# EugenHotaj/zig_gpt2

Measured on AMD Instinct MI355X. Metric: tokens/sec GPT-2-124M greedy 1024-ctx, higher is better.
Workload: dtype bf16 weights, f32 activations/accumulate; 1 GPU; GPT-2 124M greedy decode, 1 prompt(s)/GPU x 1 GPU(s), 1-token prompts, 1024 decode steps per prompt (reference generate loop, src/main.zig:322-342); vocab=50257, context=1024, n_layer=12, n_heads=12, n_embed=768, prompts_per_gpu=1, global_prompts=1, kv_cache=f32, hip_graph=True, l2_prefetcher=on, parallelism=replicated weights, prompts sharded x1, RCCL broadcast at start-up only

## Files before the change

include/zgpt2.h:

```cpp
#ifndef ZGPT2_H
#define ZGPT2_H

#include <stddef.h>
#include <stdint.h>

#ifdef __cplusplus
extern "C" {
#endif

typedef enum {
    ZG_OK = 0,
    ZG_ERR_NOT_INITIALIZED = -1,
    ZG_ERR_SHAPE = -2,
    ZG_ERR_HIP = -3,
    ZG_ERR_STAGING = -4,
    ZG_ERR_UNSUPPORTED = -5,
    ZG_ERR_ARG = -6
} zg_status;


int zg_init(int device);
int zg_init_ex(int device, size_t staging_bytes);
int zg_shutdown(void);
const char* zg_last_error(void);
// ... 36 lines not shown

int zg_gelu(float* inputs, size_t inputs_len);

int zg_softmax(float* inputs, size_t inputs_len);

int zg_gemm_bf16_nt(const uint16_t* A, const uint16_t* B, const float* bias_or_null, void* C, size_t M,
                    size_t N, size_t K, int gelu, int out_bf16);
unsigned long long zg_debug_gemm_launches(void);
int zg_debug_gemm_stamps(unsigned long long* out, size_t n_words);
int zg_debug_prefill_linear(const uint16_t* A_planes, const uint16_t* W, const float* bias_or_null, void* C, size_t M, size_t N,
                            size_t K, int epilogue, int force_kernel, int slices, float* ws, size_t ws_floats);
int zg_debug_attn_prefill(const float* qkv, uint16_t* out, size_t batch, size_t n_tokens, size_t n_embed, size_t n_heads,
                          const float* k_cache, const float* v_cache, size_t ctx, float* ws, size_t ws_floats, int key_tiles);
int zg_debug_prefill_route(int force_kernel, int slices);
int zg_debug_last_kernel(char* out, size_t n);
int zg_f32_to_bf16(const float* src, uint16_t* dst_device, size_t len);


typedef struct {
    size_t vocab_size;
    size_t context_size;
    size_t n_layer;
    size_t n_heads;
    size_t n_embed;
} zg_gpt_config;

typedef struct zg_gpt zg_gpt;

enum {
    ZG_GPT_WEIGHTS_BF16 = 0,
// ... 87 lines not shown
```

zig_gpt2_amd/_lib.py:

```python
import ctypes as C
import os
import subprocess

_HERE = os.path.dirname(os.path.abspath(__file__))
CSRC = os.path.join(_HERE, "csrc")
SO_PATH = os.environ.get("ZGPT2_LIB") or os.path.join(_HERE, "lib", "libzgpt2_hip.so")
HEADER = os.path.join(os.path.dirname(_HERE), "include", "zgpt2.h")

_lib = None

f32p = C.POINTER(C.c_float)
szp = C.POINTER(C.c_size_t)
vp = C.c_void_p
sz = C.c_size_t


class ZgError(RuntimeError):
    def __init__(self, code, msg):
        super().__init__(f"libzgpt2_hip error {code}: {msg}")
        self.code = code


class GptConfig(C.Structure):

# ... 6 lines not shown


SIGNATURES = {
    "zg_init": (C.c_int, [C.c_int]),
    "zg_init_ex": (C.c_int, [C.c_int, sz]),
    "zg_shutdown": (C.c_int, []),
    "zg_last_error": (C.c_char_p, []),
    "zg_set_stream": (C.c_int, [vp]),
    "zg_synchronize": (C.c_int, []),
    "zg_register_tensor": (C.c_int, [vp, sz]),
    "zg_unregister_tensor": (C.c_int, [vp]),
    "zg_unregister_all": (C.c_int, []),
    "zg_debug_gemm_launches": (C.c_ulonglong, []),
    "zg_debug_gemm_stamps": (C.c_int, [vp, sz]),
    "zg_debug_last_kernel": (C.c_int, [C.c_char_p, sz]),
    "zg_debug_attn_prefill": (C.c_int, [vp, vp, sz, sz, sz, sz, vp, vp, sz, vp, sz, C.c_int]),
    "zg_debug_prefill_route": (C.c_int, [C.c_int, C.c_int]),
    "zg_debug_prefill_linear": (C.c_int, [vp, vp, vp, vp, sz, sz, sz, C.c_int, C.c_int, C.c_int, vp, sz]),
    "zg_linear_forward": (C.c_int, [sz, sz, vp, vp, vp, sz, vp, sz]),
    "zg_embedding_forward": (C.c_int, [sz, vp, sz, vp, sz, vp, sz]),
    "zg_layernorm_forward": (C.c_int, [sz, vp, vp, C.c_float, vp, sz]),
    "zg_attn_forward": (C.c_int, [sz, sz, vp, vp, vp, vp, sz, vp, sz] + [vp, sz] * 8),
    "zg_split_qkv": (C.c_int, [sz, sz, vp, sz, sz, vp, sz]),
    "zg_transpose": (C.c_int, [sz, sz, sz, vp, sz, vp, sz]),
    "zg_scaled_dot_product_attention": (C.c_int, [vp, sz, vp, sz, vp, sz, sz, sz, sz, vp, sz, vp, sz]),
    "zg_gemm_bf16_nt": (C.c_int, [vp, vp, vp, vp, sz, sz, sz, C.c_int, C.c_int]),
    "zg_f32_to_bf16": (C.c_int, [vp, vp, sz]),
    "zg_gelu": (C.c_int, [vp, sz]),
    "zg_softmax": (C.c_int, [vp, sz]),
    "zg_gpt_create": (C.c_int, [C.POINTER(vp), C.POINTER(GptConfig), sz, C.c_uint]),
# ... 88 lines not shown
```

zig_gpt2_amd/csrc/api_gpt.hip:

```cpp
#include <stdio.h>
#include <stdlib.h>
#include <string.h>

#include <string>
#include <thread>
#include <vector>

#include "zg_runtime.h"

using namespace zg;

struct zg_layer {
    void *c_attn_w, *c_proj_w, *c_fc_w, *mlp_proj_w;
    bf16_t *c_attn_p, *c_proj_p, *c_fc_p, *mlp_proj_p;
    float *c_attn_c2, *c_attn_c3, *c_fc_c2, *c_fc_c3;
    float *ln_1_g, *ln_1_b, *c_attn_b, *c_proj_b, *ln_2_g, *ln_2_b, *c_fc_b, *mlp_proj_b;
    void *k_cache, *v_cache;
};

struct zg_gpt {
    zg_gpt_config cfg;
    size_t batch;
    unsigned flags;
    int wt;
// ... 18 lines not shown
    unsigned sk_epoch;
    bool sk_used;
    bf16_t *pf_a, *pf_h;
    bf16_t *xp, *hp, *ap;
    int* attn_cnt;
    unsigned* epoch;
    unsigned spin_limit;
    unsigned* fault;
    unsigned long long *sk_tag, *part_tag;
    size_t sk_tag_bytes, part_tag_bytes;
    size_t epochs_since_clear;
    bool tags_on;
    unsigned long long* qkv_tag;
    size_t qkv_tag_bytes;
    bool fused_on;
    float* xst;
    bool st_on;
    bool pl_on;
    int max_splits, lm_grid;
    StepCtrl* h_ctrl;
    int* h_ints;
    std::vector<hipGraphExec_t> graphs;
    size_t n_buckets;
    int* sampled;
    float* samp_ws;
    SampleParams* samp;
    SampleParams* h_samp;
    bool gen_sampled;
    size_t graph_steps;
    hipStream_t graph_stream;
// ... 106 lines not shown
    g->out_tokens = (int*)P(B * C * 4);
    g->sampled = (int*)P(B * 4);
    g->samp = (SampleParams*)P(sizeof(SampleParams));
    g->samp_ws = (float*)P(sample_workspace_floats((int)B) * 4);
    g->xp = (bf16_t*)P(E * 48);
    g->hp = (bf16_t*)P(4 * E * 48);
    g->ap = (bf16_t*)P(E * 48);
    g->attn_cnt = (int*)P(8 * c.n_heads * 4);
    g->epoch = (unsigned*)P(256);
    g->xst = (float*)P(((E + 15) / 16) * 8 * 2 * 4);
    g->sk_tag_bytes = ((E + 15) / 16) * 4 * 128 * 8;
    g->part_tag_bytes = 8 * c.n_heads * g->max_splits * kPartStride * 8;
    g->sk_tag = (unsigned long long*)P(g->sk_tag_bytes);
    g->qkv_tag_bytes = 3 * E * 8;
    g->qkv_tag = (unsigned long long*)P(g->qkv_tag_bytes);
    g->part_tag = (unsigned long long*)P(g->part_tag_bytes);
    g->sk_tiles = (int)((E + 15) / 16);
    g->sk_ws = (float*)P((size_t)g->sk_tiles * 4 * 128 * 4);
    g->sk_cnt = (int*)P((size_t)g->sk_tiles * 4 * 4);
    g->pf_njobs = (int)(2 + 5 * L);
    g->pf_ctl = (PfCtl*)P(sizeof(PfCtl));
    g->pf_jobs = (PfJob*)P((size_t)g->pf_njobs * sizeof(PfJob));
    g->pf_x = g->pf_qkv = g->pf_ws = nullptr;
    g->sk_flags = nullptr;
    g->sk_epoch = 0;
    g->sk_used = false;
    g->pf_a = g->pf_h = nullptr;
    g->pf_ws_floats = 0;
    if (!(g->flags & ZG_GPT_NO_PREFILL)) {
        g->pf_x = (float*)P(B * C * E * 4);
// ... 48 lines not shown
    e.vocab = (int)g->cfg.vocab_size;
    e.prompt = g->prompt;
    e.prompt_stride = (int)g->cfg.context_size;
    e.prompt_len = g->prompt_len;
    e.forced = g->forced;
    e.cur_token = g->cur_token;
    e.out_tokens = g->out_tokens;
    e.out_stride = (int)g->cfg.context_size;
    e.part_val = g->part_val;
    e.part_idx = g->part_idx;
    e.part_stride = g->lm_grid;
    e.n_partials = g->lm_grid;
    e.x = g->x;
    e.pl_out = g->pl_on ? g->xp : nullptr;
    e.pl_g = g->layers[0].ln_1_g;
    e.epoch = (((g->pl_on && g->tags_on) || g->fused_on) && finish_only != 1 && finish_only != 2) ? g->epoch : nullptr;
    e.st_out = g->st_on ? g->xst : nullptr;
    e.finish_only = finish_only;
    e.progress = g->pf_on ? &g->pf_ctl->progress : nullptr;
    e.sampled = g->sampled;
    return e;
}

int emit_gemv(const zg_gpt* g, const GemvArgs& a, int grid, hipStream_t s, std::vector<PfJob>* rec, unsigned cls) {
    if (!rec) return launch_gemv(a, g->wt, grid, s);
    PfJob j{};
    j.cls = cls;
    const int rows = gemv_rows_per_wg(a, g->wt);
    if (rows > 0) {
        j.kind = PF_WEIGHTS;
        j.base = reinterpret_cast<const char*>(a.W);
// ... 243 lines not shown
            if (rec) {
                PfJob j{};
                j.kind = PF_KV;
                j.cls = 2;
                j.base = reinterpret_cast<const char*>(y.k_cache);
                j.base2 = reinterpret_cast<const char*>(y.v_cache);
                j.n_heads = (unsigned)g->cfg.n_heads;
                j.ctx = (unsigned)g->cfg.context_size;
                j.batch = (unsigned)g->batch;
                j.row_bytes = g->kv_mode ? 128u : 256u;
                rec->push_back(j);
            } else
                ZG_TRY(launch_attn_decode(a, s));
            ZG_TRY(prof_mark(prof, 2, s));
        }
        if (only < 0 || only == 3) ZG_TRY(gemv(c_proj_args(g, y, t_hi), 3));
        if (only < 0 || only == 4) ZG_TRY(gemv(c_fc_args(g, y, t_hi), 4));
        if (only < 0 || only == 5) {
            GemvArgs a = mlp_proj_args(g, l, t_hi);
            if (a.sk_tag) a.launch_id = launch_id(l, 1);
            ZG_TRY(gemv(a, 5));
        }
    }
    if (with_logits && (only < 0 || only == 6)) {
        ZG_TRY(enqueue_lm_head(g, s, rec));
        ZG_TRY(prof_mark(prof, 6, s));
    }
    if (o.with_sampler && with_logits && only < 0 && !rec)
        ZG_TRY(launch_sample_step(g->logits, (int)g->batch, (int)g->cfg.vocab_size, g->samp, g->ctrl, g->part_val, g->lm_grid, g->lm_grid, g->samp_ws,
                                  g->sampled, s));
    return ZG_OK;
}
// ... 28 lines not shown
                                   g->pf_ws_floats, nullptr, s, nullptr, np));
        const bool more = l + 1 < L;
        const PrefillLn ln1{more ? g->layers[l + 1].ln_1_g : nullptr, more ? g->layers[l + 1].ln_1_b : nullptr, 1e-5f, g->pf_a};
        ZG_TRY(launch_prefill_gemm(g->pf_h, f32w ? y.mlp_proj_p : (const bf16_t*)y.mlp_proj_w, y.mlp_proj_b, g->pf_x, M, iE, 4 * iE, iE, PF_RESID, g->pf_ws,
                                   g->pf_ws_floats, more ? &ln1 : nullptr, s, nullptr, np));
    }
    return ZG_OK;
}

int check_fault(zg_gpt* g) {
    unsigned sk = 0, tag = 0;
    if (g->sk_used) {
        g->sk_used = false;
        ZG_TRY(gemm_s4_fault(&sk));
    }
    if (g->tags_on || g->fused_on) {
        volatile unsigned* f = g->fault;
        tag = *f;
        if (tag) *f = 0;
    }
    if (sk) {
        set_error("a half-tile hand-over of the whole-prompt c_attn GEMM timed out%s: results discarded", tag ? " (and a tagged hand-over of the decode step)" : "");
        return ZG_ERR_HIP;
    }
    if (tag) {
        set_error("a tagged hand-over of the decode step timed out (a workgroup waited %u polls for its writers): results discarded", g->spin_limit);
        return ZG_ERR_HIP;
    }
    return ZG_OK;
}

int note_steps(zg_gpt* g, size_t n, hipStream_t s) {
    if (!g->tags_on && !g->fused_on) return ZG_OK;
    g->epochs_since_clear += n;
    if (g->epochs_since_clear < ((size_t)1 << 23)) return ZG_OK;
    g->epochs_since_clear = n;
    ZG_HIP(hipMemsetAsync(g->sk_tag, 0, g->sk_tag_bytes, s));
    ZG_HIP(hipMemsetAsync(g->part_tag, 0, g->part_tag_bytes, s));
    ZG_HIP(hipMemsetAsync(g->qkv_tag, 0, g->qkv_tag_bytes, s));
    return ZG_OK;
}

int setup_prefetcher(zg_gpt* g) {
    const bool small = g->stream == nullptr && g->batch == 1 && 4 * g->cfg.n_embed * g->cfg.n_embed * g->wbytes <= ((size_t)6 << 20);
    const int want = env_int("ZGPT2_PREFETCH", small ? 1 : 0);
    if ((g->flags & ZG_GPT_NO_PREFETCH) || !want || gs(g) == nullptr) return ZG_OK;
    if (g->pf_njobs > 255) return ZG_OK;
    std::vector<PfJob> jobs;
    StepOpts describe;
    describe.rec = &jobs;
    ZG_TRY(enqueue_step(g, true, (int)g->cfg.context_size, nullptr, describe));
    ZG_REQUIRE((int)jobs.size() == g->pf_njobs, ZG_ERR_ARG, "prefetcher: %zu launches per step", jobs.size());
    ZG_HIP(hipMemcpy(g->pf_jobs, jobs.data(), jobs.size() * sizeof(PfJob), hipMemcpyHostToDevice));
    int least = 0, greatest = 0;
// ... 246 lines not shown
    }
    ZG_REQUIRE(gemv_supported(mlp_proj_args(g, 0, 0), g->wt), ZG_ERR_UNSUPPORTED,
               "batch %zu with n_embed %zu: %zu input rows of 4*n_embed floats do not fit the LDS (use a smaller batch)", batch, c.n_embed, batch);
    auto every_linear = [&](bool (*ok)(const GemvArgs&, int)) {
        return ok(c_attn_args(g, y, 0), g->wt) && ok(c_proj_args(g, y, 0), g->wt) && ok(c_fc_args(g, y, 0), g->wt) &&
               ok(mlp_proj_args(g, 0, 0), g->wt);
    };
    if (g->wt == WT_BF16 && batch >= 2 && !(decode_paths_off() & 1)) {
        g->pl_on = true;
        g->pl_on = c.n_embed % 32 == 0 && every_linear(gemv_planes_ok);
    }
    g->tags_on = g->pl_on && !(decode_paths_off() & 4);
    g->spin_limit = (unsigned)env_int("ZGPT2_TAG_SPIN_LIMIT", 1 << 20);
    g->fused_on = batch == 1 && !(decode_paths_off() & 64) && c.n_layer <= 127 &&
                  attn_qkv_ok(c_attn_args(g, y, 0), attn_args(g, y, (int)c.context_size));
    if (g->pl_on && !(decode_paths_off() & 8) && c.n_embed % 16 == 0 && c.n_embed / 16 <= 128) {
        g->st_on = true;
        g->st_on = every_linear(gemv_pl4_ok);
    }
    ZG_REQUIRE(g->lm_grid <= 4096, ZG_ERR_UNSUPPORTED, "lm_head grid %d exceeds the argmax partial buffer", g->lm_grid);
    e = hipHostMalloc(reinterpret_cast<void**>(&g->h_ctrl), sizeof(StepCtrl) + 512, hipHostMallocDefault);
    if (e == hipSuccess) e = hipHostMalloc(reinterpret_cast<void**>(&g->h_ints), (batch * c.context_size + batch) * sizeof(int), hipHostMallocDefault);
    if (e != hipSuccess) return hip_fail(e, "hipHostMalloc(control mirrors)", __FILE__, __LINE__);
    static_assert(sizeof(StepCtrl) + sizeof(SampleParams) <= 256, "the fault word sits 256 bytes behind the control mirror");
    g->h_samp = reinterpret_cast<SampleParams*>(reinterpret_cast<char*>(g->h_ctrl) + 128);
    g->fault = reinterpret_cast<unsigned*>(reinterpret_cast<char*>(g->h_ctrl) + 256);
    *g->fault = 0;
    {
        const int k = env_int("ZGPT2_GRAPH_STEPS", 8);
        g->graph_steps = (k == 2 || k == 4 || k == 8 || k == 16 || k == 32 || k == 64) ? (size_t)k : 1;
// ... 654 lines not shown
```

zig_gpt2_amd/csrc/api_ops.hip:

```cpp
#include <stdarg.h>
#include <stdio.h>
#include <stdlib.h>
#include <string.h>

#include <algorithm>

#include "zg_runtime.h"

namespace zg {

static thread_local char g_err[512] = "";

int decode_paths_off() {
    const char* e = getenv("ZGPT2_DECODE_PATHS_OFF");
    return e ? atoi(e) : 0;
}

void set_error(const char* fmt, ...) {
    va_list ap;
    va_start(ap, fmt);
    vsnprintf(g_err, sizeof(g_err), fmt, ap);
    va_end(ap);
}

static thread_local char g_kernel[160] = "";
void note_kernel(const char* fmt, ...) {
    va_list ap;
    va_start(ap, fmt);
    vsnprintf(g_kernel, sizeof(g_kernel), fmt, ap);
    va_end(ap);
}

int hip_fail(hipError_t e, const char* what, const char* file, int line) {
    set_error("HIP error %d (%s) at %s:%d: %s", (int)e, hipGetErrorString(e), file, line, what);
    (void)hipGetLastError();
    return ZG_ERR_HIP;
}

Ctx& ctx() {
    static Ctx c;
    return c;
}

int require_init() {
    ZG_REQUIRE(ctx().inited, ZG_ERR_NOT_INITIALIZED, "zg_init has not been called");
// ... 533 lines not shown

int zg_debug_prefill_route(int force_kernel, int slices) {
    ZG_REQUIRE(force_kernel >= 0 && (force_kernel <= 2 || force_kernel >= 16) && slices >= 0, ZG_ERR_ARG, "debug_prefill_route: arguments");
    prefill_force_route(force_kernel, slices);
    return ZG_OK;
}

unsigned long long zg_debug_gemm_launches(void) { return gemm_mfma_launch_count(); }
int zg_debug_gemm_stamps(unsigned long long* out, size_t n_words) { return gemm_debug_stamps(out, n_words); }
int zg_debug_last_kernel(char* out, size_t n) {
    if (!out || n == 0) return ZG_ERR_ARG;
    snprintf(out, n, "%s", zg::g_kernel);
    return ZG_OK;
}

int zg_f32_to_bf16(const float* src, uint16_t* dst_device, size_t len) {
    ZG_TRY(require_init());
    ZG_REQUIRE(src && dst_device && is_device_ptr(dst_device), ZG_ERR_ARG, "f32_to_bf16: bad argument");
    Call call;
    CallGuard guard(call);
    const float* s;
    ZG_TRY(call.in(src, len, &s));
    ZG_TRY(launch_f32_to_bf16(s, dst_device, len, call.stream()));
    ZG_TRY(call.finish());
    guard.done = true;
    return ZG_OK;
}

int zg_embedding_forward(size_t emb_dim, const float* weight, size_t weight_len, const size_t* idxs,
                         size_t idxs_len, float* embeddings, size_t embeddings_len) {
// ... 281 lines not shown
```

zig_gpt2_amd/csrc/gemv_internal.h:

```cpp
#pragma once
#include <stdlib.h>

#include "zg_kernels.h"

#ifdef ZG_STAMPS
#define ZG_STAMP_DECL() unsigned long long zg_ts[8] = {0, 0, 0, 0, 0, 0, 0, 0}
#define ZG_STAMP(i) zg_ts[i] = __builtin_amdgcn_s_memtime()
#define ZG_STAMP_FLUSH()                                                                              \
    if (a.dbg && threadIdx.x == 0 && (blockIdx.x == 0 || blockIdx.x == gridDim.x - 1)) {             \
        const unsigned long long slot = atomicAdd(a.dbg, 1ull);                                       \
        unsigned long long* d = a.dbg + 16 + slot * 10;                                               \
        for (int i = 0; i < 8; ++i) d[i] = zg_ts[i];                                                  \
        d[8] = blockIdx.x;                                                                            \
        d[9] = __builtin_amdgcn_s_memtime();                                                          \
    }
#else
#define ZG_STAMP_DECL()
#define ZG_STAMP(i)
#define ZG_STAMP_FLUSH()
#endif

namespace zg {

namespace {
// ... 358 lines not shown
    return a.kslices <= 1 && a.epilogue != EPI_ARGMAX && a.rows_per_wave == 1 && gemv_mfma_lds(a.K, 16) > 160 * 1024;
}

inline int pl4_pairs(const GemvArgs& a) {
    const int off = decode_paths_off() & 2;
    if (off || a.pl_in == nullptr || a.epilogue == EPI_ARGMAX || a.rows_per_wave != 1) return 0;
    if (a.N > 0xffff || (a.prologue == PRO_LAYERNORM && a.x_stride != a.K) || (a.epilogue == EPI_RESIDUAL && a.resid_stride != a.N)) return 0;
    if (a.st_in != nullptr && a.K / 16 > 128) return 0;
    const int ksl = a.kslices > 1 ? a.kslices : 1;
    if (a.K % (64 * ksl) != 0) return 0;
    const int kp = (a.K / ksl / 64 + 3) / 4;
    return kp <= 5 ? kp : 0;
}

template <typename WT, int LPR, int CPL, int NP, bool TAGGED>
__device__ __forceinline__ void gemv_lnk_body(int blk, const void* __restrict__ Wv, const float* __restrict__ xin, unsigned ne, int K,
                                              const float* __restrict__ ln_g, const float* __restrict__ c2, const float* __restrict__ c3,
                                              const int* __restrict__ cw, const GemvArgs& a, unsigned pf_inc,
                                              unsigned long long* __restrict__ tagw, const unsigned* __restrict__ ew, unsigned launch_id) {
    const int N = (int)(ne & 0xffffffu), epilogue = (int)(ne >> 24);
    ZG_STAMP_DECL();
    ZG_STAMP(0);
    constexpr int RPP = 64 / LPR, ROWS = NP * RPP;
    __shared__ float part[4][ROWS];
    __shared__ float stat[4][2];
    const int tid = threadIdx.x, lane = tid & 63;
    const int wave = __builtin_amdgcn_readfirstlane(tid >> 6);
    const int lr = lane % LPR, rsub = lane / LPR;
    int kbeg, nchq;
    if (sizeof(WT) == 2 && (K & 63) == 0 && ((K >> 6) & 3) != 0 && (((K >> 6) >> 2) + 1) * 8 <= LPR * CPL) {
        const int lines = K >> 6, base = lines >> 2, rem = lines & 3;
        kbeg = (wave * base + min(wave, rem)) * 64;
        nchq = (base + (wave < rem ? 1 : 0)) * 8;
    } else {
// ... 1 lines not shown
        nchq = K >> 5;
    }
    const auto W = wmat<WT>(Wv, kbeg);
    const int row0 = blk * ROWS;
    Raw<WT> wq[NP][CPL];
#pragma unroll
    for (int p = 0; p < NP; ++p) {
        const auto pr = wrow(W, (size_t)min(row0 + p * RPP + rsub, N - 1), K);
#pragma unroll
        for (int i = 0; i < CPL; ++i) wq[p][i] = load_raw(pr, min(lr + LPR * i, nchq - 1));
    }
    W8 xr[CPL], gr[CPL];
#pragma unroll
    for (int i = 0; i < CPL; ++i) {
        const size_t off = (size_t)kbeg + (size_t)min(lr + LPR * i, nchq - 1) * 8;
        xr[i] = load_x8(xin + off);
        gr[i] = load_x8(ln_g + off);
    }
    float c2n = 0.0f, c3n = 0.0f;
    if (tid < ROWS) {
        const int n = min(row0 + tid, N - 1);
        c2n = c2[n];
        c3n = c3[n];
    }
    const int T = max(cw[1], 1);
    const unsigned epoch = TAGGED ? ew[0] : 0u;
    ZG_STAMP(1);
    {
        ZG_PIN(a.progress); ZG_PIN(a.y); ZG_PIN(a.y_stride); ZG_PIN(a.epilogue); ZG_PIN(__float_as_uint(a.eps));
        if (epilogue == EPI_QKV) {
            ZG_PIN(a.q); ZG_PIN(a.k_cache); ZG_PIN(a.v_cache); ZG_PIN(a.N); ZG_PIN(a.head_dim); ZG_PIN(a.n_heads); ZG_PIN(a.ctx); ZG_PIN(a.kv_mode); ZG_PIN(a.kv_lo);
        }
    }
    if (TAGGED) { ZG_PIN(tagw); ZG_PIN(launch_id); }
    pf_count(a.progress, pf_inc);
    ZG_STAMP(2);
    float sx = 0.0f, sxx = 0.0f;
#pragma unroll
    for (int i = 0; i < CPL; ++i) {
        if (lr + LPR * i >= nchq) xr[i] = zero_w8();
#pragma unroll
        for (int j = 0; j < 8; ++j) {
            sx += xr[i].v[j];
            sxx = fmaf(xr[i].v[j], xr[i].v[j], sxx);
            xr[i].v[j] *= gr[i].v[j];
        }
    }
    sx = group_allsum<LPR>(sx);
    sxx = group_allsum<LPR>(sxx);
    auto dot = [&](const Raw<WT>(&w)[CPL]) {
// ... 59 lines not shown
```

zig_gpt2_amd/csrc/gemv_ksplit.hip:

```cpp
#include "gemv_internal.h"

namespace zg {

namespace {

template <typename WT, int LPR, int CPL, int NP = 2>
__global__ __launch_bounds__(256) void gemv_ksplit_kernel(const void* __restrict__ Wv, const float* __restrict__ xin, int N,
                                                          int K, unsigned em, const float* __restrict__ part_in, int max_splits,
                                                          const float* __restrict__ bias, const float* __restrict__ resid,
                                                          const GemvArgs a) {
    const int epilogue = (int)(em & 0xffu), merge_splits = (int)((em >> 8) & 0xffu);
    const int has_bias = (int)((em >> 16) & 1u), has_resid = (int)((em >> 17) & 1u);
    ZG_STAMP_DECL();
    ZG_STAMP(0);
    constexpr int RPP = 64 / LPR, ROWS = NP * RPP;
    __shared__ float part[4][ROWS];
    const int tid = threadIdx.x, lane = tid & 63;
    const int wave = __builtin_amdgcn_readfirstlane(tid >> 6);
    const int lr = lane % LPR, rsub = lane / LPR;
    const int Kq = K >> 2, nchq = Kq >> 3;
    const auto W = wmat<WT>(Wv, (size_t)wave * Kq);
    const int row0 = blockIdx.x * ROWS;
    Raw<WT> wq[NP][CPL];
#pragma unroll
    for (int p = 0; p < NP; ++p) {
        const auto pr = wrow(W, (size_t)min(row0 + p * RPP + rsub, N - 1), K);
#pragma unroll
        for (int i = 0; i < CPL; ++i) wq[p][i] = load_raw(pr, min(lr + LPR * i, nchq - 1));
    }
    W8 xr[CPL];
    if (merge_splits > 0) {
        constexpr int MAXS = 4;
        const int nsplit = merge_splits;
#pragma unroll
        for (int i = 0; i < CPL; ++i) {
            const int e0 = wave * Kq + min(lr + LPR * i, nchq - 1) * 8;
            const int h = e0 >> 6, d0 = e0 & 63;
            const float* p = part_in + ((size_t)h * max_splits) * kPartStride;
            float ms[MAXS], ls[MAXS];
            W8 o[MAXS];
#pragma unroll
            for (int sp = 0; sp < MAXS; ++sp) {
                const float* ps = p + min(sp, nsplit - 1) * kPartStride;
                ms[sp] = ps[64];
                ls[sp] = ps[65];
                const float2 a0 = *reinterpret_cast<const float2*>(ps + d0), a1 = *reinterpret_cast<const float2*>(ps + d0 + 2);
                const float2 a2 = *reinterpret_cast<const float2*>(ps + d0 + 4), a3 = *reinterpret_cast<const float2*>(ps + d0 + 6);
                o[sp].v[0] = a0.x; o[sp].v[1] = a0.y; o[sp].v[2] = a1.x; o[sp].v[3] = a1.y;
                o[sp].v[4] = a2.x; o[sp].v[5] = a2.y; o[sp].v[6] = a3.x; o[sp].v[7] = a3.y;
            }
#pragma unroll
            for (int sp = 0; sp < MAXS; ++sp)
                if (sp >= nsplit) ms[sp] = -1e30f;
            const float mx = fmaxf(fmaxf(ms[0], ms[1]), fmaxf(ms[2], ms[3]));
            float l = 0.0f;
            W8 r = zero_w8();
#pragma unroll
            for (int sp = 0; sp < MAXS; ++sp) {
                const float w = __expf(ms[sp] - mx);
                l = fmaf(w, ls[sp], l);
#pragma unroll
                for (int j = 0; j < 8; ++j) r.v[j] = fmaf(w, o[sp].v[j], r.v[j]);
            }
            const float inv = 1.0f / l;
#pragma unroll
            for (int j = 0; j < 8; ++j) xr[i].v[j] = r.v[j] * inv;
        }
    } else {
#pragma unroll
        for (int i = 0; i < CPL; ++i) xr[i] = load_x8(xin + (size_t)wave * Kq + (size_t)min(lr + LPR * i, nchq - 1) * 8);
    }
    float bias_n = 0.0f, resid_n = 0.0f;
    if (tid < ROWS) {
        const int n = min(row0 + tid, N - 1);
        bias_n = bias[n * has_bias];
        resid_n = resid[n * has_resid];
    }
    ZG_STAMP(1);
    ZG_PIN(a.y);
    ZG_PIN(a.progress);
    pf_count(a.progress);
    ZG_STAMP(2);
#pragma unroll
    for (int i = 0; i < CPL; ++i)
        if (lr + LPR * i >= nchq) xr[i] = zero_w8();
    auto dot = [&](const Raw<WT>(&w)[CPL]) {
        float p0 = 0.0f, p1 = 0.0f, p2 = 0.0f, p3 = 0.0f;
#pragma unroll
        for (int i = 0; i < CPL; ++i) {
            const W8 u = unpack(w[i]);
            p0 = fmaf(u.v[0], xr[i].v[0], p0); p1 = fmaf(u.v[1], xr[i].v[1], p1);
            p2 = fmaf(u.v[2], xr[i].v[2], p2); p3 = fmaf(u.v[3], xr[i].v[3], p3);
            p0 = fmaf(u.v[4], xr[i].v[4], p0); p1 = fmaf(u.v[5], xr[i].v[5], p1);
            p2 = fmaf(u.v[6], xr[i].v[6], p2); p3 = fmaf(u.v[7], xr[i].v[7], p3);
        }
        return group_allsum<LPR>((p0 + p1) + (p2 + p3));
    };
    float sp[NP];
#pragma unroll
    for (int p = 0; p < NP; ++p) sp[p] = dot(wq[p]);
    ZG_STAMP(3);
    if (lr == 0) {
#pragma unroll
        for (int p = 0; p < NP; ++p) part[wave][p * RPP + rsub] = sp[p];
    }
    __syncthreads();
    ZG_STAMP(4);
    if (tid < ROWS && row0 + tid < N) {
        const int n = row0 + tid;
        const float v = ((part[0][tid] + part[1][tid]) + (part[2][tid] + part[3][tid])) + bias_n;
        a.y[n] = epilogue == EPI_RESIDUAL ? v + resid_n : (epilogue == EPI_GELU ? gelu_ref(v) : v);
    }
    ZG_STAMP(5);
    ZG_STAMP(6);
    ZG_STAMP(7);
    ZG_STAMP_FLUSH();
}

template <typename WT>
int launch_ksplit(const GemvArgs& a, hipStream_t s) {
    const int nchq = a.K / 32;
    const int merge_splits = a.prologue == PRO_ATTN_MERGE ? (a.t_hi + kAttnChunk - 1) / kAttnChunk : 0;
    const unsigned has_resid = a.epilogue == EPI_RESIDUAL ? 1u : 0u;
    const unsigned em = (unsigned)a.epilogue | ((unsigned)merge_splits << 8) | ((a.bias ? 1u : 0u) << 16) | (has_resid << 17);
#define ZG_KS(LPR_, CPL_)                                                                                                \
    {                                                                                                                    \
        constexpr int rows = 2 * (64 / LPR_);                                                                            \
        note_kernel("gemv_ksplit_kernel<%s, %d, %d, 2>", wt_name<WT>(), LPR_, CPL_);         \
        hipLaunchKernelGGL((gemv_ksplit_kernel<WT, LPR_, CPL_, 2>), dim3((a.N + rows - 1) / rows), dim3(256), 0, s, a.W,     \
                           a.x,                                                                                         \
                           a.N, a.K, em, a.part ? a.part : a.zero, a.max_splits, a.bias ? a.bias : a.zero,              \
// ... 111 lines not shown
```

zig_gpt2_amd/csrc/zg_kernels.h:

```cpp
#pragma once
#include "zg_common.h"

namespace zg {

struct StepCtrl {
    int step;
    int seq_len;
    int mode;
    int n_partials;
};

enum GemvPrologue { PRO_NONE = 0, PRO_LAYERNORM = 1, PRO_ATTN_MERGE = 2 };
enum GemvEpilogue { EPI_STORE = 0, EPI_RESIDUAL = 1, EPI_GELU = 2, EPI_QKV = 3, EPI_ARGMAX = 4 };
enum WeightType { WT_BF16 = 0, WT_F32 = 1, WT_B24 = 2  };

constexpr int kAttnChunk = 256;
constexpr int kPartStride = 64 + 2;

struct GemvArgs {
    const void* W;
    const float* bias;
    int N, K, M;
    int rows_per_wave;
    int waves_per_wg;
// ... 66 lines not shown
    int t_hi;
    int max_splits;
    float* part;
    unsigned* progress;
    bf16_t* pl_out;
    int* merge_cnt;
    const unsigned* epoch;
    unsigned launch_id;
    unsigned long long* part_tag;
    unsigned* fault;
    unsigned spin_limit;
};
int launch_attn_decode(const AttnArgs& a, hipStream_t s);
bool attn_qkv_ok(const GemvArgs& g, const AttnArgs& at);
int launch_attn_qkv(const GemvArgs& g, int weight_type, const AttnArgs& at, const unsigned* epoch, unsigned long long* qkv_tag, hipStream_t s);
int launch_attn_any_dim(const float* q, const float* k, const float* v, long stride_b, long stride_h, long stride_t, int batch, int n_heads,
                        int head_dim, int seq_len, float* out, hipStream_t s);
int launch_attn_merge(const float* part, int batch, int n_heads, int head_dim, int max_splits,
                      int seq_len, float* out, hipStream_t s);

int launch_epoch_bump(unsigned* epoch, hipStream_t s);
int launch_layernorm(float* x, int rows, int n, const float* g, const float* b, float eps, hipStream_t s, unsigned* done_flag = nullptr,
                     unsigned done_seq = 0, bool* announced = nullptr, float* shadow = nullptr);
int launch_gelu(float* x, size_t n, hipStream_t s, unsigned* done_flag = nullptr, unsigned done_seq = 0, bool* announced = nullptr, float* shadow = nullptr);
int launch_softmax(float* x, size_t n, hipStream_t s, unsigned* done_flag = nullptr, unsigned done_seq = 0, bool* announced = nullptr);
int launch_done_flag(unsigned* flag, unsigned seq, hipStream_t s);
struct CopySegs {
    const void* src[4];
    void* dst[4];
    unsigned bytes[4];
// ... 165 lines not shown
```

Before: 5021 tokens/s.

## Fuse attention c_proj and MLP c_fc gemvs into one tagged launch

Adds a combined kernel in which the first blocks compute the attention output projection with residual and publish each output element with an epoch/launch tag. The remaining blocks run the layernorm+c_fc+GELU gemv, preload their weights, then spin on the tags instead of waiting for a kernel boundary. This removes one launch and one inter-kernel gap per layer and lets c_fc weight loads overlap c_proj. In exchange it relies on both block groups being co-resident, with a spin limit and fault flag as the fallback. Also factors the ksplit gemv body into a shared device function and adds a per-name kernel launch counter for debugging.

New measurement: 5016 tokens/s. Within noise of the previous version (-0.1%).

```diff
diff --git a/include/zgpt2.h b/include/zgpt2.h
--- a/include/zgpt2.h
+++ b/include/zgpt2.h
@@ -74,6 +74,7 @@
                           const float* k_cache, const float* v_cache, size_t ctx, float* ws, size_t ws_floats, int key_tiles);
 int zg_debug_prefill_route(int force_kernel, int slices);
 int zg_debug_last_kernel(char* out, size_t n);
+unsigned long long zg_debug_kernel_launches(const char* prefix);
 int zg_f32_to_bf16(const float* src, uint16_t* dst_device, size_t len);
 
 
diff --git a/zig_gpt2_amd/_lib.py b/zig_gpt2_amd/_lib.py
--- a/zig_gpt2_amd/_lib.py
+++ b/zig_gpt2_amd/_lib.py
@@ -44,6 +44,7 @@
     "zg_debug_gemm_launches": (C.c_ulonglong, []),
     "zg_debug_gemm_stamps": (C.c_int, [vp, sz]),
     "zg_debug_last_kernel": (C.c_int, [C.c_char_p, sz]),
+    "zg_debug_kernel_launches": (C.c_ulonglong, [C.c_char_p]),
     "zg_debug_attn_prefill": (C.c_int, [vp, vp, sz, sz, sz, sz, vp, vp, sz, vp, sz, C.c_int]),
     "zg_debug_prefill_route": (C.c_int, [C.c_int, C.c_int]),
     "zg_debug_prefill_linear": (C.c_int, [vp, vp, vp, vp, sz, sz, sz, C.c_int, C.c_int, C.c_int, vp, sz]),
diff --git a/zig_gpt2_amd/csrc/api_gpt.hip b/zig_gpt2_amd/csrc/api_gpt.hip
--- a/zig_gpt2_amd/csrc/api_gpt.hip
+++ b/zig_gpt2_amd/csrc/api_gpt.hip
@@ -56,6 +56,9 @@
     unsigned long long* qkv_tag;
     size_t qkv_tag_bytes;
     bool fused_on;
+    unsigned long long* x_tag;
+    size_t x_tag_bytes;
+    bool projfc_on;
     float* xst;
     bool st_on;
     bool pl_on;
@@ -192,6 +195,8 @@
     g->sk_tag = (unsigned long long*)P(g->sk_tag_bytes);
     g->qkv_tag_bytes = 3 * E * 8;
     g->qkv_tag = (unsigned long long*)P(g->qkv_tag_bytes);
+    g->x_tag_bytes = E * 8;
+    g->x_tag = (unsigned long long*)P(g->x_tag_bytes);
     g->part_tag = (unsigned long long*)P(g->part_tag_bytes);
     g->sk_tiles = (int)((E + 15) / 16);
     g->sk_ws = (float*)P((size_t)g->sk_tiles * 4 * 128 * 4);
@@ -270,7 +275,7 @@
     e.x = g->x;
     e.pl_out = g->pl_on ? g->xp : nullptr;
     e.pl_g = g->layers[0].ln_1_g;
-    e.epoch = (((g->pl_on && g->tags_on) || g->fused_on) && finish_only != 1 && finish_only != 2) ? g->epoch : nullptr;
+    e.epoch = (((g->pl_on && g->tags_on) || g->fused_on || g->projfc_on) && finish_only != 1 && finish_only != 2) ? g->epoch : nullptr;
     e.st_out = g->st_on ? g->xst : nullptr;
     e.finish_only = finish_only;
     e.progress = g->pf_on ? &g->pf_ctl->progress : nullptr;
@@ -544,8 +549,18 @@
                 ZG_TRY(launch_attn_decode(a, s));
             ZG_TRY(prof_mark(prof, 2, s));
         }
-        if (only < 0 || only == 3) ZG_TRY(gemv(c_proj_args(g, y, t_hi), 3));
-        if (only < 0 || only == 4) ZG_TRY(gemv(c_fc_args(g, y, t_hi), 4));
+        bool pf = false;
+        if (g->projfc_on && !g->pf_on && only < 0 && !rec && 2 * l + 1 <= 255) {
+            const GemvArgs p = c_proj_args(g, y, t_hi), c = c_fc_args(g, y, t_hi);
+            if (proj_fc_ok(p, c)) {
+                pf = true;
+                ZG_TRY(launch_proj_fc(p, c, g->wt, g->epoch, g->x_tag, g->fault, g->spin_limit, launch_id(l, 0), s));
+                ZG_TRY(prof_mark(prof, 3, s));
+                ZG_TRY(prof_mark(prof, 4, s));
+            }
+        }
+        if (!pf && (only < 0 || only == 3)) ZG_TRY(gemv(c_proj_args(g, y, t_hi), 3));
+        if (!pf && (only < 0 || only == 4)) ZG_TRY(gemv(c_fc_args(g, y, t_hi), 4));
         if (only < 0 || only == 5) {
             GemvArgs a = mlp_proj_args(g, l, t_hi);
             if (a.sk_tag) a.launch_id = launch_id(l, 1);
@@ -604,7 +619,7 @@
         g->sk_used = false;
         ZG_TRY(gemm_s4_fault(&sk));
     }
-    if (g->tags_on || g->fused_on) {
+    if (g->tags_on || g->fused_on || g->projfc_on) {
         volatile unsigned* f = g->fault;
         tag = *f;
         if (tag) *f = 0;
@@ -621,13 +636,14 @@
 }
 
 int note_steps(zg_gpt* g, size_t n, hipStream_t s) {
-    if (!g->tags_on && !g->fused_on) return ZG_OK;
+    if (!g->tags_on && !g->fused_on && !g->projfc_on) return ZG_OK;
     g->epochs_since_clear += n;
     if (g->epochs_since_clear < ((size_t)1 << 23)) return ZG_OK;
     g->epochs_since_clear = n;
     ZG_HIP(hipMemsetAsync(g->sk_tag, 0, g->sk_tag_bytes, s));
     ZG_HIP(hipMemsetAsync(g->part_tag, 0, g->part_tag_bytes, s));
     ZG_HIP(hipMemsetAsync(g->qkv_tag, 0, g->qkv_tag_bytes, s));
+    ZG_HIP(hipMemsetAsync(g->x_tag, 0, g->x_tag_bytes, s));
     return ZG_OK;
 }
 
@@ -904,6 +920,7 @@
     g->spin_limit = (unsigned)env_int("ZGPT2_TAG_SPIN_LIMIT", 1 << 20);
     g->fused_on = batch == 1 && !(decode_paths_off() & 64) && c.n_layer <= 127 &&
                   attn_qkv_ok(c_attn_args(g, y, 0), attn_args(g, y, (int)c.context_size));
+    g->projfc_on = batch == 1 && !(decode_paths_off() & 128) && c.n_layer <= 127 && proj_fc_ok(c_proj_args(g, y, 64), c_fc_args(g, y, 64));
     if (g->pl_on && !(decode_paths_off() & 8) && c.n_embed % 16 == 0 && c.n_embed / 16 <= 128) {
         g->st_on = true;
         g->st_on = every_linear(gemv_pl4_ok);
diff --git a/zig_gpt2_amd/csrc/api_ops.hip b/zig_gpt2_amd/csrc/api_ops.hip
--- a/zig_gpt2_amd/csrc/api_ops.hip
+++ b/zig_gpt2_amd/csrc/api_ops.hip
@@ -24,11 +24,23 @@
 }
 
 static thread_local char g_kernel[160] = "";
+struct KernelCount {
+    char name[160];
+    unsigned long long n;
+};
+static thread_local KernelCount g_kernel_counts[64];
 void note_kernel(const char* fmt, ...) {
     va_list ap;
     va_start(ap, fmt);
     vsnprintf(g_kernel, sizeof(g_kernel), fmt, ap);
     va_end(ap);
+    for (KernelCount& k : g_kernel_counts) {
+        if (k.n == 0) memcpy(k.name, g_kernel, sizeof(k.name));
+        if (strcmp(k.name, g_kernel) == 0) {
+            ++k.n;
+            break;
+        }
+    }
 }
 
 int hip_fail(hipError_t e, const char* what, const char* file, int line) {
@@ -592,6 +604,14 @@
     return ZG_OK;
 }
 
+unsigned long long zg_debug_kernel_launches(const char* prefix) {
+    unsigned long long n = 0;
+    if (prefix)
+        for (const zg::KernelCount& k : zg::g_kernel_counts)
+            if (k.n && strncmp(k.name, prefix, strlen(prefix)) == 0) n += k.n;
+    return n;
+}
+
 int zg_f32_to_bf16(const float* src, uint16_t* dst_device, size_t len) {
     ZG_TRY(require_init());
     ZG_REQUIRE(src && dst_device && is_device_ptr(dst_device), ZG_ERR_ARG, "f32_to_bf16: bad argument");
diff --git a/zig_gpt2_amd/csrc/gemv_internal.h b/zig_gpt2_amd/csrc/gemv_internal.h
--- a/zig_gpt2_amd/csrc/gemv_internal.h
+++ b/zig_gpt2_amd/csrc/gemv_internal.h
@@ -396,10 +396,131 @@
 }
 
 template <typename WT, int LPR, int CPL, int NP, bool TAGGED>
+__device__ __forceinline__ void gemv_ksplit_body(int blk, const void* __restrict__ Wv, const float* __restrict__ xin, int N, int K, unsigned em,
+                                                 const float* __restrict__ part_in, int max_splits, const float* __restrict__ bias,
+                                                 const float* __restrict__ resid, const GemvArgs& a, unsigned pf_inc,
+                                                 unsigned long long* __restrict__ tagw, const unsigned* __restrict__ ew, unsigned launch_id) {
+    const int epilogue = (int)(em & 0xffu), merge_splits = (int)((em >> 8) & 0xffu);
+    const int has_bias = (int)((em >> 16) & 1u), has_resid = (int)((em >> 17) & 1u);
+    ZG_STAMP_DECL();
+    ZG_STAMP(0);
+    constexpr int RPP = 64 / LPR, ROWS = NP * RPP;
+    __shared__ float part[4][ROWS];
+    const int tid = threadIdx.x, lane = tid & 63;
+    const int wave = __builtin_amdgcn_readfirstlane(tid >> 6);
+    const int lr = lane % LPR, rsub = lane / LPR;
+    const int Kq = K >> 2, nchq = Kq >> 3;
+    const auto W = wmat<WT>(Wv, (size_t)wave * Kq);
+    const int row0 = (int)((unsigned)blk * (unsigned)ROWS);
+    Raw<WT> wq[NP][CPL];
+#pragma unroll
+    for (int p = 0; p < NP; ++p) {
+        const auto pr = wrow(W, (size_t)min(row0 + p * RPP + rsub, N - 1), K);
+#pragma unroll
+        for (int i = 0; i < CPL; ++i) wq[p][i] = load_raw(pr, min(lr + LPR * i, nchq - 1));
+    }
+    W8 xr[CPL];
+    if (merge_splits > 0) {
+        constexpr int MAXS = 4;
+        const int nsplit = merge_splits;
+#pragma unroll
+        for (int i = 0; i < CPL; ++i) {
+            const int e0 = wave * Kq + min(lr + LPR * i, nchq - 1) * 8;
+            const int h = e0 >> 6, d0 = e0 & 63;
+            const float* p = part_in + ((size_t)h * max_splits) * kPartStride;
+            float ms[MAXS], ls[MAXS];
+            W8 o[MAXS];
+#pragma unroll
+            for (int sp = 0; sp < MAXS; ++sp) {
+                const float* ps = p + min(sp, nsplit - 1) * kPartStride;
+                ms[sp] = ps[64];
+                ls[sp] = ps[65];
+                const float2 a0 = *reinterpret_cast<const float2*>(ps + d0), a1 = *reinterpret_cast<const float2*>(ps + d0 + 2);
+                const float2 a2 = *reinterpret_cast<const float2*>(ps + d0 + 4), a3 = *reinterpret_cast<const float2*>(ps + d0 + 6);
+                o[sp].v[0] = a0.x; o[sp].v[1] = a0.y; o[sp].v[2] = a1.x; o[sp].v[3] = a1.y;
+                o[sp].v[4] = a2.x; o[sp].v[5] = a2.y; o[sp].v[6] = a3.x; o[sp].v[7] = a3.y;
+            }
+#pragma unroll
+            for (int sp = 0; sp < MAXS; ++sp)
+                if (sp >= nsplit) ms[sp] = -1e30f;
+            const float mx = fmaxf(fmaxf(ms[0], ms[1]), fmaxf(ms[2], ms[3]));
+            float l = 0.0f;
+            W8 r = zero_w8();
+#pragma unroll
+            for (int sp = 0; sp < MAXS; ++sp) {
+                const float w = __expf(ms[sp] - mx);
+                l = fmaf(w, ls[sp], l);
+#pragma unroll
+                for (int j = 0; j < 8; ++j) r.v[j] = fmaf(w, o[sp].v[j], r.v[j]);
+            }
+            const float inv = 1.0f / l;
+#pragma unroll
+            for (int j = 0; j < 8; ++j) xr[i].v[j] = r.v[j] * inv;
+        }
+    } else {
+#pragma unroll
+        for (int i = 0; i < CPL; ++i) xr[i] = load_x8(xin + (size_t)wave * Kq + (size_t)min(lr + LPR * i, nchq - 1) * 8);
+    }
+    float bias_n = 0.0f, resid_n = 0.0f;
+    if (tid < ROWS) {
+        const int n = min(row0 + tid, N - 1);
+        bias_n = bias[n * has_bias];
+        resid_n = resid[n * has_resid];
+    }
+    const unsigned epoch = TAGGED ? ew[0] : 0u;
+    ZG_STAMP(1);
+    ZG_PIN(a.y);
+    ZG_PIN(a.progress);
+    if (TAGGED) { ZG_PIN(tagw); ZG_PIN(launch_id); }
+    pf_count(a.progress, pf_inc);
+    ZG_STAMP(2);
+#pragma unroll
+    for (int i = 0; i < CPL; ++i)
+        if (lr + LPR * i >= nchq) xr[i] = zero_w8();
+    auto dot = [&](const Raw<WT>(&w)[CPL]) {
+        float p0 = 0.0f, p1 = 0.0f, p2 = 0.0f, p3 = 0.0f;
+#pragma unroll
+        for (int i = 0; i < CPL; ++i) {
+            const W8 u = unpack(w[i]);
+            p0 = fmaf(u.v[0], xr[i].v[0], p0); p1 = fmaf(u.v[1], xr[i].v[1], p1);
+            p2 = fmaf(u.v[2], xr[i].v[2], p2); p3 = fmaf(u.v[3], xr[i].v[3], p3);
+            p0 = fmaf(u.v[4], xr[i].v[4], p0); p1 = fmaf(u.v[5], xr[i].v[5], p1);
+            p2 = fmaf(u.v[6], xr[i].v[6], p2); p3 = fmaf(u.v[7], xr[i].v[7], p3);
+        }
+        return group_allsum<LPR>((p0 + p1) + (p2 + p3));
+    };
+    float sp[NP];
+#pragma unroll
+    for (int p = 0; p < NP; ++p) sp[p] = dot(wq[p]);
+    ZG_STAMP(3);
+    if (lr == 0) {
+#pragma unroll
+        for (int p = 0; p < NP; ++p) part[wave][p * RPP + rsub] = sp[p];
+    }
+    __syncthreads();
+    ZG_STAMP(4);
+    if (tid < ROWS && row0 + tid < N) {
+        const int n = row0 + tid;
+        const float v = ((part[0][tid] + part[1][tid]) + (part[2][tid] + part[3][tid])) + bias_n;
+        const float out = epilogue == EPI_RESIDUAL ? v + resid_n : (epilogue == EPI_GELU ? gelu_ref(v) : v);
+        a.y[n] = out;
+        if (TAGGED)
+            __hip_atomic_store(tagw + n, ((unsigned long long)((epoch << 8) | launch_id) << 32) | __float_as_uint(out), __ATOMIC_RELAXED,
+                               __HIP_MEMORY_SCOPE_AGENT);
+    }
+    ZG_STAMP(5);
+    ZG_STAMP(6);
+    ZG_STAMP(7);
+    ZG_STAMP_FLUSH();
+}
+
+template <typename WT, int LPR, int CPL, int NP, bool TAGGED, bool XT = false>
 __device__ __forceinline__ void gemv_lnk_body(int blk, const void* __restrict__ Wv, const float* __restrict__ xin, unsigned ne, int K,
                                               const float* __restrict__ ln_g, const float* __restrict__ c2, const float* __restrict__ c3,
                                               const int* __restrict__ cw, const GemvArgs& a, unsigned pf_inc,
-                                              unsigned long long* __restrict__ tagw, const unsigned* __restrict__ ew, unsigned launch_id) {
+                                              unsigned long long* __restrict__ tagw, const unsigned* __restrict__ ew, unsigned launch_id,
+                                              const unsigned long long* __restrict__ xtag = nullptr, unsigned xid = 0u,
+                                              unsigned* __restrict__ fault = nullptr, unsigned spin_limit = 0u) {
     const int N = (int)(ne & 0xffffffu), epilogue = (int)(ne >> 24);
     ZG_STAMP_DECL();
     ZG_STAMP(0);
@@ -431,7 +552,7 @@
 #pragma unroll
     for (int i = 0; i < CPL; ++i) {
         const size_t off = (size_t)kbeg + (size_t)min(lr + LPR * i, nchq - 1) * 8;
-        xr[i] = load_x8(xin + off);
+        if (!XT) xr[i] = load_x8(xin + off);
         gr[i] = load_x8(ln_g + off);
     }
     float c2n = 0.0f, c3n = 0.0f;
@@ -441,7 +562,7 @@
         c3n = c3[n];
     }
     const int T = max(cw[1], 1);
-    const unsigned epoch = TAGGED ? ew[0] : 0u;
+    const unsigned epoch = (TAGGED || XT) ? ew[0] : 0u;
     ZG_STAMP(1);
     {
         ZG_PIN(a.progress); ZG_PIN(a.y); ZG_PIN(a.y_stride); ZG_PIN(a.epilogue); ZG_PIN(__float_as_uint(a.eps));
@@ -451,6 +572,39 @@
     }
     if (TAGGED) { ZG_PIN(tagw); ZG_PIN(launch_id); }
     pf_count(a.progress, pf_inc);
+    if constexpr (XT) {
+        constexpr int QW = LPR * CPL * 8, NX = QW / 64;
+        __shared__ __attribute__((aligned(16))) float xs[4][QW];
+        ZG_PIN(xtag); ZG_PIN(xid); ZG_PIN(fault); ZG_PIN(spin_limit);
+        const unsigned tag = (epoch << 8) | xid;
+        const int nw = nchq * 8;
+        const unsigned long long* src = xtag + kbeg;
+        unsigned long long wv[NX];
+#pragma unroll
+        for (int j = 0; j < NX; ++j) wv[j] = 0ull;
+        for (unsigned spins = 0;; ++spins) {
+            bool ok = true;
+#pragma unroll
+            for (int j = 0; j < NX; ++j) {
+                if (64 * j < nw) {
+                    wv[j] = __hip_atomic_load(src + min(lane + 64 * j, nw - 1), __ATOMIC_RELAXED, __HIP_MEMORY_SCOPE_AGENT);
+                    ok = ok && (unsigned)(wv[j] >> 32) == tag;
+                }
+            }
+            if (__builtin_amdgcn_ballot_w64(!ok) == 0) break;
+            if (spins >= spin_limit) {
+                if (lane == 0 && fault) __hip_atomic_store(fault, 1u, __ATOMIC_RELAXED, __HIP_MEMORY_SCOPE_AGENT);
+                break;
+            }
+            __builtin_amdgcn_s_sleep(1);
+        }
+#pragma unroll
+        for (int j = 0; j < NX; ++j)
+            if (lane + 64 * j < nw) xs[wave][lane + 64 * j] = __uint_as_float((unsigned)wv[j]);
+        __builtin_amdgcn_wave_barrier();
+#pragma unroll
+        for (int i = 0; i < CPL; ++i) xr[i] = load_x8(&xs[wave][min(lr + LPR * i, nchq - 1) * 8]);
+    }
     ZG_STAMP(2);
     float sx = 0.0f, sxx = 0.0f;
 #pragma unroll
diff --git a/zig_gpt2_amd/csrc/gemv_ksplit.hip b/zig_gpt2_amd/csrc/gemv_ksplit.hip
--- a/zig_gpt2_amd/csrc/gemv_ksplit.hip
+++ b/zig_gpt2_amd/csrc/gemv_ksplit.hip
@@ -9,112 +9,7 @@
                                                           int K, unsigned em, const float* __restrict__ part_in, int max_splits,
                                                           const float* __restrict__ bias, const float* __restrict__ resid,
                                                           const GemvArgs a) {
-    const int epilogue = (int)(em & 0xffu), merge_splits = (int)((em >> 8) & 0xffu);
-    const int has_bias = (int)((em >> 16) & 1u), has_resid = (int)((em >> 17) & 1u);
-    ZG_STAMP_DECL();
-    ZG_STAMP(0);
-    constexpr int RPP = 64 / LPR, ROWS = NP * RPP;
-    __shared__ float part[4][ROWS];
-    const int tid = threadIdx.x, lane = tid & 63;
-    const int wave = __builtin_amdgcn_readfirstlane(tid >> 6);
-    const int lr = lane % LPR, rsub = lane / LPR;
-    const int Kq = K >> 2, nchq = Kq >> 3;
-    const auto W = wmat<WT>(Wv, (size_t)wave * Kq);
-    const int row0 = blockIdx.x * ROWS;
-    Raw<WT> wq[NP][CPL];
-#pragma unroll
-    for (int p = 0; p < NP; ++p) {
-        const auto pr = wrow(W, (size_t)min(row0 + p * RPP + rsub, N - 1), K);
-#pragma unroll
-        for (int i = 0; i < CPL; ++i) wq[p][i] = load_raw(pr, min(lr + LPR * i, nchq - 1));
-    }
-    W8 xr[CPL];
-    if (merge_splits > 0) {
-        constexpr int MAXS = 4;
-        const int nsplit = merge_splits;
-#pragma unroll
-        for (int i = 0; i < CPL; ++i) {
-            const int e0 = wave * Kq + min(lr + LPR * i, nchq - 1) * 8;
-            const int h = e0 >> 6, d0 = e0 & 63;
-            const float* p = part_in + ((size_t)h * max_splits) * kPartStride;
-            float ms[MAXS], ls[MAXS];
-            W8 o[MAXS];
-#pragma unroll
-            for (int sp = 0; sp < MAXS; ++sp) {
-                const float* ps = p + min(sp, nsplit - 1) * kPartStride;
-                ms[sp] = ps[64];
-                ls[sp] = ps[65];
-                const float2 a0 = *reinterpret_cast<const float2*>(ps + d0), a1 = *reinterpret_cast<const float2*>(ps + d0 + 2);
-                const float2 a2 = *reinterpret_cast<const float2*>(ps + d0 + 4), a3 = *reinterpret_cast<const float2*>(ps + d0 + 6);
-                o[sp].v[0] = a0.x; o[sp].v[1] = a0.y; o[sp].v[2] = a1.x; o[sp].v[3] = a1.y;
-                o[sp].v[4] = a2.x; o[sp].v[5] = a2.y; o[sp].v[6] = a3.x; o[sp].v[7] = a3.y;
-            }
-#pragma unroll
-            for (int sp = 0; sp < MAXS; ++sp)
-                if (sp >= nsplit) ms[sp] = -1e30f;
-            const float mx = fmaxf(fmaxf(ms[0], ms[1]), fmaxf(ms[2], ms[3]));
-            float l = 0.0f;
-            W8 r = zero_w8();
-#pragma unroll
-            for (int sp = 0; sp < MAXS; ++sp) {
-                const float w = __expf(ms[sp] - mx);
-                l = fmaf(w, ls[sp], l);
-#pragma unroll
-                for (int j = 0; j < 8; ++j) r.v[j] = fmaf(w, o[sp].v[j], r.v[j]);
-            }
-            const float inv = 1.0f / l;
-#pragma unroll
-            for (int j = 0; j < 8; ++j) xr[i].v[j] = r.v[j] * inv;
-        }
-    } else {
-#pragma unroll
-        for (int i = 0; i < CPL; ++i) xr[i] = load_x8(xin + (size_t)wave * Kq + (size_t)min(lr + LPR * i, nchq - 1) * 8);
-    }
-    float bias_n = 0.0f, resid_n = 0.0f;
-    if (tid < ROWS) {
-        const int n = min(row0 + tid, N - 1);
-        bias_n = bias[n * has_bias];
-        resid_n = resid[n * has_resid];
-    }
-    ZG_STAMP(1);
-    ZG_PIN(a.y);
-    ZG_PIN(a.progress);
-    pf_count(a.progress);
-    ZG_STAMP(2);
-#pragma unroll
-    for (int i = 0; i < CPL; ++i)
-        if (lr + LPR * i >= nchq) xr[i] = zero_w8();
-    auto dot = [&](const Raw<WT>(&w)[CPL]) {
-        float p0 = 0.0f, p1 = 0.0f, p2 = 0.0f, p3 = 0.0f;
-#pragma unroll
-        for (int i = 0; i < CPL; ++i) {
-            const W8 u = unpack(w[i]);
-            p0 = fmaf(u.v[0], xr[i].v[0], p0); p1 = fmaf(u.v[1], xr[i].v[1], p1);
-            p2 = fmaf(u.v[2], xr[i].v[2], p2); p3 = fmaf(u.v[3], xr[i].v[3], p3);
-            p0 = fmaf(u.v[4], xr[i].v[4], p0); p1 = fmaf(u.v[5], xr[i].v[5], p1);
-            p2 = fmaf(u.v[6], xr[i].v[6], p2); p3 = fmaf(u.v[7], xr[i].v[7], p3);
-        }
-        return group_allsum<LPR>((p0 + p1) + (p2 + p3));
-    };
-    float sp[NP];
-#pragma unroll
-    for (int p = 0; p < NP; ++p) sp[p] = dot(wq[p]);
-    ZG_STAMP(3);
-    if (lr == 0) {
-#pragma unroll
-        for (int p = 0; p < NP; ++p) part[wave][p * RPP + rsub] = sp[p];
-    }
-    __syncthreads();
-    ZG_STAMP(4);
-    if (tid < ROWS && row0 + tid < N) {
-        const int n = row0 + tid;
-        const float v = ((part[0][tid] + part[1][tid]) + (part[2][tid] + part[3][tid])) + bias_n;
-        a.y[n] = epilogue == EPI_RESIDUAL ? v + resid_n : (epilogue == EPI_GELU ? gelu_ref(v) : v);
-    }
-    ZG_STAMP(5);
-    ZG_STAMP(6);
-    ZG_STAMP(7);
-    ZG_STAMP_FLUSH();
+    gemv_ksplit_body<WT, LPR, CPL, NP, false>((int)blockIdx.x, Wv, xin, N, K, em, part_in, max_splits, bias, resid, a, 1u, nullptr, nullptr, 0u);
 }
 
 template <typename WT>
diff --git a/zig_gpt2_amd/csrc/proj_fc.hip b/zig_gpt2_amd/csrc/proj_fc.hip
--- /dev/null
+++ b/zig_gpt2_amd/csrc/proj_fc.hip
@@ -0,0 +1,77 @@
+#include "gemv_internal.h"
+
+namespace zg {
+
+namespace {
+
+struct ProjFcArgs {
+    const float* ln_g;
+    const float* c2;
+    const float* c3;
+    const int* cw;
+    const unsigned* ew;
+    unsigned long long* x_tag;
+    unsigned* fault;
+    unsigned spin_limit, launch_id;
+};
+
+constexpr int kLpr = 16, kCpl = 2, kProjRows = 2 * (64 / kLpr), kFcRows = 4 * (64 / kLpr);
+
+template <typename WT>
+__global__ __launch_bounds__(256) void proj_fc_kernel(const void* __restrict__ Wp, const float* __restrict__ part_in, const float* __restrict__ bias,
+                                                      const float* __restrict__ resid, const void* __restrict__ Wf, int E, unsigned em,
+                                                      int max_splits, unsigned ne, const GemvArgs a, const GemvArgs c, const ProjFcArgs f) {
+    const unsigned blk = blockIdx.x;
+    const unsigned G = ((unsigned)E + kProjRows - 1) / kProjRows, A0 = (G + 7u) & ~7u;
+    if (blk < G) {
+        gemv_ksplit_body<WT, kLpr, kCpl, 2, true>((int)blk, Wp, nullptr, E, E, em, part_in, max_splits, bias, resid, a, 2u, f.x_tag, f.ew,
+                                                  f.launch_id);
+        return;
+    }
+    if (blk < A0) return;
+    gemv_lnk_body<WT, kLpr, kCpl, 4, false, true>((int)(blk - A0), Wf, nullptr, ne, E, f.ln_g, f.c2, f.c3, f.cw, c, 0u, nullptr, f.ew, 0u, f.x_tag,
+                                                  f.launch_id, f.fault, f.spin_limit);
+}
+
+}
+
+bool proj_fc_ok(const GemvArgs& p, const GemvArgs& c) {
+    if (p.part == nullptr || p.resid == nullptr || p.y == nullptr) return false;
+    if (!gemv_use_ksplit(p) || p.prologue != PRO_ATTN_MERGE || p.epilogue != EPI_RESIDUAL || p.M != 1 || p.N != p.K || p.K / 32 > kLpr * kCpl) return false;
+    if (!gemv_use_lnk(c) || c.epilogue != EPI_GELU || c.M != 1 || c.K != p.N || c.x != p.y || c.y == nullptr || c.N > 0xffffff) return false;
+    return p.pl_in == nullptr && p.pl_out == nullptr && c.pl_in == nullptr && c.pl_out == nullptr && c.st_in == nullptr && p.st_out == nullptr &&
+           c.ctrl != nullptr;
+}
+
+int launch_proj_fc(const GemvArgs& p, const GemvArgs& c, int weight_type, const unsigned* epoch, unsigned long long* x_tag, unsigned* fault,
+                   unsigned spin_limit, unsigned launch_id, hipStream_t s) {
+    ZG_REQUIRE(proj_fc_ok(p, c) && epoch != nullptr && x_tag != nullptr && launch_id >= 1 && launch_id <= 255, ZG_ERR_ARG,
+               "fused c_proj + c_fc: unsupported arguments");
+    const int merge_splits = (p.t_hi + kAttnChunk - 1) / kAttnChunk;
+    const unsigned em = (unsigned)p.epilogue | ((unsigned)merge_splits << 8) | ((p.bias ? 1u : 0u) << 16) | (1u << 17);
+    ProjFcArgs f{};
+    f.ln_g = c.ln_g;
+    f.c2 = c.ln_c2;
+    f.c3 = c.ln_c3;
+    f.cw = reinterpret_cast<const int*>(c.ctrl);
+    f.ew = epoch;
+    f.x_tag = x_tag;
+    f.fault = fault;
+    f.spin_limit = spin_limit;
+    f.launch_id = launch_id;
+    const unsigned G = (unsigned)((p.N + kProjRows - 1) / kProjRows), A0 = (G + 7u) & ~7u;
+    const unsigned grid = A0 + (unsigned)((c.N + kFcRows - 1) / kFcRows);
+    const unsigned ne = (unsigned)c.N | ((unsigned)c.epilogue << 24);
+    note_kernel("proj_fc_kernel<%s>", weight_type == WT_BF16 ? "unsigned short" : weight_type == WT_B24 ? "b24" : "float");
+#define ZG_PF(WT_)                                                                                                                              \
+    hipLaunchKernelGGL((proj_fc_kernel<WT_>), dim3(grid), dim3(256), 0, s, p.W, p.part, p.bias ? p.bias : p.zero, p.resid, c.W, p.N, em, p.max_splits, \
+                       ne, p, c, f)
+    if (weight_type == WT_BF16) ZG_PF(bf16_t);
+    else if (weight_type == WT_B24) ZG_PF(b24_t);
+    else ZG_PF(float);
+#undef ZG_PF
+    ZG_HIP(hipGetLastError());
+    return ZG_OK;
+}
+
+}
diff --git a/zig_gpt2_amd/csrc/zg_kernels.h b/zig_gpt2_amd/csrc/zg_kernels.h
--- a/zig_gpt2_amd/csrc/zg_kernels.h
+++ b/zig_gpt2_amd/csrc/zg_kernels.h
@@ -104,6 +104,9 @@
 int launch_attn_decode(const AttnArgs& a, hipStream_t s);
 bool attn_qkv_ok(const GemvArgs& g, const AttnArgs& at);
 int launch_attn_qkv(const GemvArgs& g, int weight_type, const AttnArgs& at, const unsigned* epoch, unsigned long long* qkv_tag, hipStream_t s);
+bool proj_fc_ok(const GemvArgs& p, const GemvArgs& c);
+int launch_proj_fc(const GemvArgs& p, const GemvArgs& c, int weight_type, const unsigned* epoch, unsigned long long* x_tag, unsigned* fault,
+                   unsigned spin_limit, unsigned launch_id, hipStream_t s);
 int launch_attn_any_dim(const float* q, const float* k, const float* v, long stride_b, long stride_h, long stride_t, int batch, int n_heads,
                         int head_dim, int seq_len, float* out, hipStream_t s);
 int launch_attn_merge(const float* part, int batch, int n_heads, int head_dim, int max_splits,
```
